# musevlt/origin

Measured on AMD Instinct MI355X. Metric: voxels/s through DCT+PCA+GLR (ORIGIN hot path), higher is better.
Workload: dtype f32+f16x2; 1 GPU; synthetic 3681x600x600 cube, Dico_FWHM_2_12 (20 profiles), PSF 25x25, 100x100 areas, dct_order 10, pfa 0.01, Noise_population 50, itermax 100; masked_border=0, glr_spectral_arithmetic=f16x2, tiles=1

## Files before the change

origin_amd/csrc/glr.hip:

```cpp
#include <algorithm>

#include "glr_plan.h"

namespace {

__global__ __launch_bounds__(256) void maxmap_final_kernel(const float *__restrict__ part_max,
                                                           const float *__restrict__ part_min,
                                                           int nzc, long S,
                                                           float *__restrict__ maxmap,
                                                           float *__restrict__ minmap) {
  const long s = (long)blockIdx.x * 256 + threadIdx.x;
  if (s >= S) return;
  float a = -INFINITY, b = INFINITY;
  for (int k = 0; k < nzc; ++k) {
    a = fmaxf(a, part_max[(long)k * S + s]);
    b = fminf(b, part_min[(long)k * S + s]);
  }
  if (maxmap) maxmap[s] = a;
  if (minmap) minmap[s] = b;
}

int launch_maxmap_final(origin_ctx *ctx, const GlrSpectralIO &io, long S, float *d_maxmap,
                        float *d_minmap) {
  hipLaunchKernelGGL(maxmap_final_kernel, dim3(cdiv(S, 256)), dim3(256), 0, ctx->stream, io.pmax,
// ... 32 lines not shown
                  GlrSpectralIO *io) {
  io->nzc = glr_part_rows(ctx, pl, form);
  io->pmax = io->want_maps ? io->part : nullptr;
  io->pmin = io->want_maps ? io->part + (size_t)io->nzc * pl->Ny * pl->Nx : nullptr;
}

int run_spectral_mfma(origin_ctx *ctx, const origin_glr_plan *pl, GlrSpectral form, bool no_fold,
                      GlrSpectralIO *io, const GlrRange &rg) {
  lay_out_maps(ctx, pl, form, io);
  if (form == GLR_SPEC_NORM_MFMA) return origin_spectral_norm_mfma_launch(ctx, pl, *io, rg);
  const bool normw = form == GLR_SPEC_NORMW;
  SpectralMfmaArgs a = glr_spectral_mfma_args(pl, io, normw || !no_fold);
  a.range = rg;
  if (!normw) return origin_spectral_mfma_launch(ctx, a);
  a.rden = a.rdi_s = a.rden_fold = a.sden = nullptr;
  a.normc = io->norm;
  if (int rc = origin_spectral_mfma_launch(ctx, a)) return rc;
  return origin_spectral_norm_mfma_launch_ends(ctx, pl, *io, rg,
                                               glr_part_rows(ctx, pl, GLR_SPEC_TABLE));
}

}

SpectralMfmaArgs glr_spectral_mfma_args(const origin_glr_plan *pl, const GlrSpectralIO *io,
                                        bool fold) {
  const bool b16 = pl->precision == 2;
  SpectralMfmaArgs a;
  a.io = io;
  a.terms = b16 ? 1 : 3;
  a.atab = b16 ? pl->d_atab_bf16 : pl->d_atab;
  a.atab_fold = !fold ? nullptr : b16 ? pl->d_atab_bf16_fold : pl->d_atab_fold;
  a.rden = pl->d_rden, a.rdi_s = pl->d_rdi_s;
  a.rden_fold = fold ? pl->d_rden_fold : nullptr, a.sden = fold ? pl->d_sden : nullptr;
  a.pinfo = pl->d_pwide;
  a.NzP = pl->NzP, a.K = pl->K, a.n_narrow = pl->n_narrow, a.ident = pl->order_ident;
  a.Nz = pl->Nz, a.Ny = pl->Ny, a.Nx = pl->Nx, a.P = pl->P;
  return a;
}

extern "C" {

int origin_glr_run_rows(origin_ctx *ctx, origin_glr_plan *pl, const float *d_cube,
                        const uint8_t *d_mask, float *d_work, float *d_correl, uint8_t *d_profile,
                        float *d_correl_min, int y0, int y1, int flags) {
  return origin_glr_run_rect(ctx, pl, d_cube, d_mask, d_work, d_correl, d_profile, d_correl_min, y0,
                             y1, 0, pl ? pl->Nx : 0, flags);
}

int origin_glr_run_rect(origin_ctx *ctx, origin_glr_plan *pl, const float *d_cube,
                        const uint8_t *d_mask, float *d_work, float *d_correl, uint8_t *d_profile,
                        float *d_correl_min, int y0, int y1, int x0, int x1, int flags) {
  ORIGIN_USE(ctx);
  ORIGIN_CHECK_ARG(pl && pl->ctx == ctx, "plan does not belong to this context");
  ORIGIN_CHECK_ARG(d_cube && d_work && d_correl && d_profile && d_correl_min, "null pointer");
  const int Ny = pl->Ny, Nx = pl->Nx;
  ORIGIN_CHECK_ARG(y0 >= 0 && y0 < y1 && y1 <= Ny && y0 % 64 == 0 && (y1 % 64 == 0 || y1 == Ny),
                   "row band must start at a multiple of 64 and end at one or at Ny");
  ORIGIN_CHECK_ARG(x0 >= 0 && x0 < x1 && x1 <= Nx && x0 % 64 == 0 && (x1 % 64 == 0 || x1 == Nx),
                   "column range must start at a multiple of 64 and end at one or at Nx");
  const bool no_fold = glr_no_fold();
  const GlrPaths paths = glr_paths(pl, no_fold);
  if (!paths.prepared) {
    origin_set_error("origin_glr_run_rows: a plan with a norm cube runs in bands after "
                     "origin_glr_plan_prepare");
    return ORIGIN_E_STATE;
  }
  if (!paths.rows_ok()) {
    origin_set_error("origin_glr_run_rows: the plan's stages do not run the matrix-core kernels");
// ... 74 lines not shown
```

origin_amd/csrc/glr_plan.h:

```cpp
#pragma once
#include <cmath>
#include <cstdlib>
#include <vector>

#include "common.h"
#include "glr_tables.h"

struct origin_glr_plan {
  origin_ctx *ctx = nullptr;
  int Nz = 0, Ny = 0, Nx = 0, nfields = 0, P = 0, K = 0;
  int mode = 0;
  int lwmax = 0;
  float *d_k = nullptr;
  float *d_k2 = nullptr;
  float *d_w = nullptr;
  float *d_taps = nullptr;
  float *d_taps2 = nullptr;
  int *d_tap_off = nullptr;
  float *d_rden = nullptr;
  int Kp = 0;
  int symmetric = 0;
  float *d_htaps = nullptr;
  int *d_htap_off = nullptr;
  float *d_rows = nullptr;
  float *d_rdi = nullptr;
  int *d_border = nullptr;
  int nborder = 0;
  int lwt = 0;
  int NzP = 0;
  uint4 *d_atab = nullptr;
  uint4 *d_atab_bf16 = nullptr;
  uint4 *d_atab2 = nullptr;
  int *d_pwide = nullptr;
  int n_narrow = 0;
  int order_ident = 0;
  float *d_rdi_s = nullptr;
  uint4 *d_atab_fold = nullptr, *d_atab_bf16_fold = nullptr;
  float *d_rden_fold = nullptr, *d_sden = nullptr;
  float fold_eps = INFINITY;
  int normw_checked = 0;
  std::vector<int> h_order;
  int precision = 0;
  float *d_normc = nullptr;
  int normc_ready = 0;
  size_t bytes = 0;
};

enum GlrSpectral {
  GLR_SPEC_TABLE,
  GLR_SPEC_NORMW,
  GLR_SPEC_NORM_MFMA,
  GLR_SPEC_PACKED,
  GLR_SPEC_FP32,
  GLR_SPEC_GENERIC
};
struct GlrPaths {
  bool spatial_mfma;
  GlrSpectral spectral;
  bool prepared;
  bool spectral_mfma() const { return spectral <= GLR_SPEC_NORM_MFMA; }
  bool rows_ok() const { return prepared && spatial_mfma && spectral_mfma(); }
};
inline bool glr_no_fold() { return getenv("ORIGIN_GLR_NO_FOLD") != nullptr; }
GlrPaths glr_paths_at(const origin_glr_plan *pl, int precision, bool no_fold);
inline GlrPaths glr_paths(const origin_glr_plan *pl, bool no_fold) {
  return glr_paths_at(pl, pl->precision, no_fold);
}

// ... 15 lines not shown

int glr_fp32_spatial(origin_ctx *ctx, const float *A, const float *B, const float *taps, int Nz,
                     int Ny, int Nx, int P, int accumulate, float *out);
struct GlrSpectralIO {
  const float *fsf, *norm;
  const uint8_t *mask;
  float *correl;
  uint8_t *profile;
  float *correl_min;
  float *part;
  bool want_maps;
  int nzc = 0;
  float *pmax = nullptr, *pmin = nullptr;
};
int glr_fp32_spectral(origin_ctx *ctx, const origin_glr_plan *pl, GlrSpectral form,
                      GlrSpectralIO *io, ProfScope *ps);
int glr_fp32_border_maps(origin_ctx *ctx, const origin_glr_plan *pl, const float *correl,
                         const float *correl_min, float *maxmap, float *minmap);

struct GlrRange {
  int y0 = 0, y1 = 0, x0 = 0, x1 = 0;
};
struct GlrSpaxels {
  long s_first, s_end, bx;
  int rx0, rx1;
};
int glr_range_resolve(const GlrRange &rg, int Ny, int Nx, int waves, GlrSpaxels *sp);
struct GlrChunks {
  int n, len;
};
GlrChunks glr_z_chunks(int num_cu, int Nz, long S, int waves);
int glr_part_rows(const origin_ctx *ctx, const origin_glr_plan *pl, GlrSpectral form);

struct SpectralMfmaArgs {
  const GlrSpectralIO *io;
  int terms;
  const uint4 *atab, *atab_fold;
  const float *rden, *rdi_s, *rden_fold, *sden;
  const int *pinfo;
  int NzP, K, n_narrow, ident;
  int Nz, Ny, Nx, P;
  GlrRange range;
  const float *normc = nullptr;
};
SpectralMfmaArgs glr_spectral_mfma_args(const origin_glr_plan *pl, const GlrSpectralIO *io,
                                        bool fold);
int origin_spectral_mfma_launch(origin_ctx *ctx, const SpectralMfmaArgs &a);
long origin_spectral_mfma_count(int num_cu, int terms, int K, int n_narrow, int Nz, int Ny,
                                int Nx);

int origin_spectral_norm_mfma_max_k();
int origin_spectral_norm_mfma_launch(origin_ctx *ctx, const origin_glr_plan *pl,
                                     const GlrSpectralIO &io, const GlrRange &rg);
int origin_spectral_norm_mfma_launch_ends(origin_ctx *ctx, const origin_glr_plan *pl,
                                          const GlrSpectralIO &io, const GlrRange &rg, int prow0);
```

origin_amd/csrc/glr_plan.hip:

```cpp
#include <algorithm>
#include <cmath>
#include <cstdlib>
#include <memory>
#include <vector>

#include "glr_plan.h"

namespace {

__global__ __launch_bounds__(256) void norm_classes_kernel(const float *__restrict__ k2, int Nz,
                                                           int P, double *__restrict__ ncls) {
  const long i = (long)blockIdx.x * 256 + threadIdx.x;
  const long n = (long)Nz * P * P;
  if (i >= n) return;
  const int z = (int)(i / (P * P));
  const int cls = (int)(i - (long)z * P * P);
  const int cy = cls / P, cx = cls - cy * P;
  const int c = P / 2;
  const int dy0 = max(0, c - cy), dy1 = min(P - 1, P - 1 + c - cy);
  const int dx0 = max(0, c - cx), dx1 = min(P - 1, P - 1 + c - cx);
  const float *kz = k2 + (long)z * P * P;
  double acc = 0.0;
  for (int dy = dy0; dy <= dy1; ++dy)
    for (int dx = dx0; dx <= dx1; ++dx) acc += (double)kz[dy * P + dx];
// ... 251 lines not shown
  };
  for (int slot = 0; slot < K; ++slot) {
    const int kk = order[slot];
    const int L = prof.len(kk), lw = prof.lw(kk);
    pinfo[slot] = kk | ((lw > 16) << 8);
    for (int c = 0; c < 8; ++c)
      for (int q = 0; q < MF_GROUPS; ++q)
        for (int j = 0; j < 8; ++j) {
          const int e = 8 * q + c + j, ti = lw + 63 - e;
          const float t = (ti >= 0 && ti < L) ? prof.taps[prof.off[kk] + ti] : 0.0f;
          const size_t base = slot * PROF + c * COPY + (size_t)q * 8 + j;
          split(t * tscale, &at[base]);
          ab[base] = to_bf16(t);
          if (!atf.empty()) {
            const float tf = (float)((double)t * (*fold_a)[kk]);
            split(tf * tscale, &atf[base]);
            abf[base] = to_bf16(tf);
          }
          if (!at2.empty()) split((t * t) * tscale, &at2[base]);
        }
  }
  origin_ctx *ctx = pl->ctx;
  if (int rc = upload(ctx, at, (_Float16 **)&pl->d_atab, &pl->bytes)) return rc;
  if (int rc = upload(ctx, ab, (unsigned short **)&pl->d_atab_bf16, &pl->bytes)) return rc;
  if (!at2.empty())
    if (int rc = upload(ctx, at2, (_Float16 **)&pl->d_atab2, &pl->bytes)) return rc;
  if (!atf.empty()) {
    if (int rc = upload(ctx, atf, (_Float16 **)&pl->d_atab_fold, &pl->bytes)) return rc;
    if (int rc = upload(ctx, abf, (unsigned short **)&pl->d_atab_bf16_fold, &pl->bytes)) return rc;
  }
  if (int rc = upload(ctx, pinfo, &pl->d_pwide, &pl->bytes)) return rc;
  pl->n_narrow = 0;
  for (int slot = 0; slot < K; ++slot) pl->n_narrow += (pinfo[slot] >> 8) == 0;
  pl->order_ident = 1;
  for (int slot = 0; slot < K; ++slot) pl->order_ident &= order[slot] == slot;
  pl->h_order = order;
  return ORIGIN_OK;
}

int alloc_norm_cube(origin_glr_plan *pl) {
  const size_t padded =
      ((size_t)pl->Nz + MF_PAD_FRONT + MF_PAD_BACK) * (size_t)pl->Ny * pl->Nx * sizeof(float);
  ORIGIN_HIP(hipMalloc((void **)&pl->d_normc, padded));
  ORIGIN_HIP(hipMemsetAsync(pl->d_normc, 0, padded, pl->ctx->stream));
  pl->bytes += padded;
  return ORIGIN_OK;
}

int build_border_tables(origin_glr_plan *pl) {
  origin_ctx *ctx = pl->ctx;
  const int Nz = pl->Nz, Ny = pl->Ny, Nx = pl->Nx, P = pl->P, K = pl->K, NzP = pl->NzP;
  const size_t PP = (size_t)P * P;
  std::vector<int> border;
  const int c = P / 2;
  for (int y = 0; y < Ny; ++y)
    for (int x = 0; x < Nx; ++x)
      if (y < c || y > Ny - 1 - c || x < c || x > Nx - 1 - c) border.push_back(y * Nx + x);
  pl->nborder = (int)border.size();
  if (int rc = upload(ctx, border, &pl->d_border, &pl->bytes)) return rc;
  DevTmp ncls;
  const size_t ncls_n = (size_t)Nz * PP, rn = PP * (size_t)K * NzP;
  ORIGIN_HIP(ncls.alloc(ncls_n * sizeof(double)));
  ORIGIN_HIP(hipMalloc((void **)&pl->d_rden, rn * sizeof(float)));
  pl->bytes += rn * sizeof(float);
  hipLaunchKernelGGL(norm_classes_kernel, dim3(cdiv((long)ncls_n, 256)), dim3(256), 0, ctx->stream,
                     pl->d_k2, Nz, P, (double *)ncls.p);
  hipLaunchKernelGGL(rden_kernel, dim3(cdiv((long)rn, 256)), dim3(256), 0, ctx->stream,
                     (const double *)ncls.p, pl->d_taps2, pl->d_tap_off, K, Nz, (int)PP, NzP,
// ... 145 lines not shown
  float *norm = pl->d_normc + (size_t)MF_PAD_FRONT * S;
  if (!pl->normc_ready) {
    ProfScope ps(ctx, K_GLR_SPATIAL);
    for (int f = 0; f < pl->nfields; ++f) {
      const float *wf = pl->d_w ? pl->d_w + (size_t)f * S : nullptr;
      const float *k2f = pl->d_k2 + (size_t)f * Nz * P * P;
      if (int rc = glr_fp32_spatial(ctx, nullptr, wf, k2f, Nz, Ny, Nx, P, f > 0, norm)) return rc;
    }
    pl->normc_ready = 1;
  }
  if (!pl->normw_checked) {
    if (pl->d_atab_fold) return measure_normw_eps(ctx, pl, norm);
    pl->normw_checked = 1;
  }
  return ORIGIN_OK;
}

extern "C" {

int origin_glr_plan_prepare(origin_ctx *ctx, origin_glr_plan *plan) {
  ORIGIN_USE(ctx);
  ORIGIN_CHECK_ARG(plan && plan->ctx == ctx, "plan does not belong to this context");
  return glr_plan_prepare(ctx, plan);
}

int origin_glr_plan_destroy(origin_glr_plan *plan) {
  if (!plan) return ORIGIN_OK;
  (void)hipSetDevice(plan->ctx->device);
  (void)hipStreamSynchronize(plan->ctx->stream);
  for (void *p : {(void *)plan->d_k, (void *)plan->d_k2, (void *)plan->d_w, (void *)plan->d_taps,
                  (void *)plan->d_taps2, (void *)plan->d_tap_off, (void *)plan->d_rden,
                  (void *)plan->d_htaps, (void *)plan->d_htap_off, (void *)plan->d_rows,
                  (void *)plan->d_border, (void *)plan->d_atab, (void *)plan->d_atab_bf16,
                  (void *)plan->d_pwide, (void *)plan->d_rdi_s, (void *)plan->d_normc,
                  (void *)plan->d_atab2, (void *)plan->d_atab_fold, (void *)plan->d_atab_bf16_fold,
                  (void *)plan->d_rden_fold, (void *)plan->d_sden})
    if (p) (void)hipFree(p);
  delete plan;
  return ORIGIN_OK;
}

int origin_glr_plan_create(origin_ctx *ctx, int Nz, int Ny, int Nx, int nfields, int P,
                           const double *h_psf, const double *h_weights, int K,
                           const double *h_taps, const int *h_tap_off,
                           origin_glr_plan **out) {
  ORIGIN_USE(ctx);
  ORIGIN_CHECK_ARG(out, "out is null");
  *out = nullptr;
  ORIGIN_CHECK_ARG(Nz > 0 && Ny > 0 && Nx > 0, "bad cube shape (%d,%d,%d)", Nz, Ny, Nx);
  ORIGIN_CHECK_ARG(nfields >= 1 && h_psf, "need at least one PSF");
  ORIGIN_CHECK_ARG(P >= 1 && (P & 1) && P <= 63, "PSF size %d unsupported (odd, <= 63)", P);
  ORIGIN_CHECK_ARG(K >= 1 && K <= 255 && h_taps && h_tap_off,
                   "need 1..255 profiles (profile index is uint8)");
  ORIGIN_CHECK_ARG(h_weights || nfields == 1, "several fields need weight maps");
  for (int k = 0; k < K; ++k)
    ORIGIN_CHECK_ARG(h_tap_off[k + 1] > h_tap_off[k], "profile %d is empty", k);

  std::unique_ptr<origin_glr_plan, PlanDeleter> owner(new origin_glr_plan());
  origin_glr_plan *pl = owner.get();
  pl->ctx = ctx;
  pl->Nz = Nz, pl->Ny = Ny, pl->Nx = Nx, pl->nfields = nfields, pl->P = P, pl->K = K;
  pl->mode = (h_weights == nullptr && Ny >= P && Nx >= P) ? 0 : 1;
  pl->NzP = (Nz + 31) / 32 * 32 + 32;
  pl->Kp = pl->NzP;

  Profiles prof;
  std::vector<double> fold_a;
// ... 18 lines not shown

int origin_glr_plan_set_precision(origin_glr_plan *plan, int precision) {
  ORIGIN_CHECK_ARG(plan && precision >= 0 && precision <= 2, "precision must be 0, 1 or 2");
  const GlrPaths at1 = glr_paths_at(plan, 1, false);
  plan->precision = at1.spatial_mfma || at1.spectral_mfma() ? precision : 0;
  return ORIGIN_OK;
}

int origin_glr_plan_get_precision(origin_glr_plan *plan, int *precision) {
  ORIGIN_CHECK_ARG(plan && precision, "null argument");
  *precision = plan->precision;
  return ORIGIN_OK;
}

int origin_glr_plan_fold_eps(origin_glr_plan *plan, float *eps, int *active) {
  ORIGIN_CHECK_ARG(plan && eps && active, "null argument");
  *eps = plan->fold_eps;
  *active = (plan->mode == 0 ? plan->d_rden_fold != nullptr
                             : plan->normw_checked && plan->d_atab_fold != nullptr &&
                                   plan->fold_eps <= MF_FOLD_EPS) &&
            !glr_no_fold();
  return ORIGIN_OK;
}

int origin_glr_plan_mfma_count(origin_glr_plan *plan, long *spatial, long *spectral) {
  ORIGIN_CHECK_ARG(plan && spatial && spectral, "null argument");
  const origin_glr_plan *pl = plan;
  *spatial = *spectral = 0;
  const GlrPaths paths = glr_paths(pl, glr_no_fold());
  const int terms = pl->precision == 2 ? 1 : 3;
  if (pl->mode == 0 && paths.spatial_mfma)
    *spatial = origin_spatial_mfma_count(terms, pl->Nz, pl->Ny, pl->Nx, pl->P);
  if (paths.spectral == GLR_SPEC_TABLE)
    *spectral = origin_spectral_mfma_count(pl->ctx->num_cu, terms, pl->K, pl->n_narrow, pl->Nz,
                                           pl->Ny, pl->Nx);
  return ORIGIN_OK;
}

int origin_glr_mfma_count_model(int num_cu, int terms, int K, int n_narrow, int Nz, int Ny, int Nx,
                                int P, long *spatial, long *spectral) {
  ORIGIN_CHECK_ARG(spatial && spectral && num_cu > 0 && (terms == 1 || terms == 3) && K > 0 &&
                       n_narrow >= 0 && n_narrow <= K && Nz > 0 && Ny > 0 && Nx > 0 && P > 0,
                   "bad arguments");
  *spatial = origin_spatial_mfma_ok(Ny, Nx, P) ? origin_spatial_mfma_count(terms, Nz, Ny, Nx, P) : 0;
  *spectral = origin_spectral_mfma_count(num_cu, terms, K, n_narrow, Nz, Ny, Nx);
  return ORIGIN_OK;
}

int origin_glr_plan_paths(origin_glr_plan *plan, int *spatial_mfma, int *spectral, int *lwt,
                          int *lwmax, int *nborder) {
  ORIGIN_CHECK_ARG(plan && spatial_mfma && spectral && lwt && lwmax && nborder, "null argument");
  const GlrPaths paths = glr_paths(plan, glr_no_fold());
  *spatial_mfma = paths.spatial_mfma ? 1 : 0;
  *spectral = (int)paths.spectral;
  *lwt = plan->lwt;
  *lwmax = plan->lwmax;
  *nborder = plan->nborder;
  return ORIGIN_OK;
}

int origin_glr_plan_bytes(origin_glr_plan *plan, size_t *bytes) {
  ORIGIN_CHECK_ARG(plan && bytes, "null argument");
  *bytes = plan->bytes;
  return ORIGIN_OK;
}

int origin_glr_work_elems(origin_glr_plan *plan, size_t *elems) {
  ORIGIN_CHECK_ARG(plan && elems, "null argument");
  *elems = GlrWork::elems(plan);
  return ORIGIN_OK;
}

int origin_glr_rows_supported(origin_glr_plan *plan, int *ok) {
  ORIGIN_CHECK_ARG(plan && ok, "null argument");
  *ok = glr_paths(plan, glr_no_fold()).rows_ok() ? 1 : 0;
  return ORIGIN_OK;
}

// ... 2 lines not shown
```

origin_amd/csrc/glr_spectral_mfma.hip:

```cpp
#include <algorithm>

#include "glr_plan.h"

namespace {

constexpr bool SM_PREFETCH = MF_WAVES <= 8;

#ifdef SM_TIMING
__device__ long long sm_wave[4 * MF_WAVES * 3];
__device__ long long sm_tim[8 * MF_WAVES * 8];
#define SM_STAMP(k)                                                                       \
  if (blockIdx.x == 3 && blockIdx.y == 1 && lane == 0 && sm_tile >= 2 && sm_tile < 10)    \
  sm_tim[((sm_tile - 2) * MF_WAVES + (threadIdx.x >> 6)) * 8 + (k)] = clock64()
#else
#define SM_STAMP(k)
#endif

typedef unsigned u32x4v __attribute__((ext_vector_type(4)));
typedef float f32x16 __attribute__((ext_vector_type(16)));
typedef float f32x4v __attribute__((ext_vector_type(4)));
typedef _Float16 f16x2v __attribute__((ext_vector_type(2)));

template <int I, int N, typename F>
__device__ __forceinline__ void sm_for(F &&f) {
// ... 47 lines not shown
        : "v"(acc[O]), "v"(acc[O + 8]), "v"(maskv), "s"(ca), "s"(cb), "s"(ninf), "s"(pinf));
    return;
  }
  if constexpr (FOLD) {
    asm volatile(
        "v_and_or_b32 %0, %5, %7, %8\n\t"
        "v_and_or_b32 %1, %6, %7, %9\n\t"
        "v_max3_f32 %2, %2, %0, %1\n\t"
        "v_max3_f32 %3, %3, %5, %6\n\t"
        "v_min3_f32 %4, %4, %5, %6"
        : "=&v"(K0), "=&v"(K1), "+v"(st.key[O]), "+v"(st.best[O]), "+v"(st.worst[O])
        : "v"(acc[O]), "v"(acc[O + 8]), "v"(maskv), "s"(ca), "s"(cb));
    return;
  }
  asm volatile(
      "v_mul_f32 %0, %7, %8\n\t"
      "v_mul_f32 %1, %9, %10\n\t"
      "v_and_or_b32 %2, %0, %11, %12\n\t"
      "v_and_or_b32 %3, %1, %11, %13\n\t"
      "v_max3_f32 %4, %4, %2, %3\n\t"
      "v_max3_f32 %5, %5, %0, %1\n\t"
      "v_min3_f32 %6, %6, %0, %1"
      : "=&v"(T0), "=&v"(T1), "=&v"(K0), "=&v"(K1), "+v"(st.key[O]), "+v"(st.best[O]),
        "+v"(st.worst[O])
      : "v"(acc[O]), "v"(fa[g][q]), "v"(acc[O + 8]), "v"(fb[g][q]), "v"(maskv), "s"(ca), "s"(cb));
}

constexpr int SM_EPI_ITEMS = 8;

constexpr int sm_epi_start(int j, int NM) {
  return j < 2 ? 0 : (j >= NM ? SM_EPI_ITEMS : (SM_EPI_ITEMS * (j - 2)) / (NM - 2));
}

template <int TERMS, int OFF, bool FOLD, int MODE = EPI_UPDATE>
__device__ __forceinline__ void sm_stage(const char *ak, const char *ak_next, u32x4v &fh,
                                         u32x4v &fl, bool wide, const u32x4v (&bh)[6],
                                         const u32x4v (&bl)[6], f32x16 &acc, const f32x16 &pacc,
                                         const f32x4v (&pfa)[2], const f32x4v (&pfb)[2],
                                         SmState &st, unsigned maskv, int pca, int pcb) {
  constexpr int LO = 8 * MF_COPY_BYTES;
  constexpr int NM = TERMS * 3;
  u32x4v ah, al;
  if constexpr (FOLD) {
    ah = fh, al = fl;
  } else {
    ah = *reinterpret_cast<const u32x4v *>(ak + 32), al = ah;
    if constexpr (TERMS == 3) al = *reinterpret_cast<const u32x4v *>(ak + 32 + LO);
  }
  sm_for<0, 3>([&](auto ic) {
    constexpr int g = decltype(ic)::value, ks = 1 + g;
    u32x4v nh = ah, nl = al;
    if constexpr (g + 1 < 3) {
      nh = *reinterpret_cast<const u32x4v *>(ak + (ks + 1) * 32);
      if constexpr (TERMS == 3) nl = *reinterpret_cast<const u32x4v *>(ak + (ks + 1) * 32 + LO);
    } else if constexpr (FOLD) {
      nh = *reinterpret_cast<const u32x4v *>(ak_next + 32), nl = nh;
      if constexpr (TERMS == 3) nl = *reinterpret_cast<const u32x4v *>(ak_next + 32 + LO);
    }
    auto gap = [&](auto jc) {
      constexpr int j = decltype(jc)::value;
      sm_for<sm_epi_start(j, NM), sm_epi_start(j + 1, NM)>([&](auto kc) {
        sm_epi_item<decltype(kc)::value, FOLD, MODE>(pacc, pfa, pfb, st, maskv, pca, pcb);
      });
    };
    sm_mma<TERMS, g == 0>(acc, ah, bh[OFF + ks]);
    gap(std::integral_constant<int, TERMS * g>{});
    if constexpr (TERMS == 3) {
      sm_mma<TERMS, false>(acc, ah, bl[OFF + ks]);
      gap(std::integral_constant<int, TERMS * g + 1>{});
      sm_mma<TERMS, false>(acc, al, bh[OFF + ks]);
      gap(std::integral_constant<int, TERMS * g + 2>{});
    }
    ah = nh, al = nl;
  });
  if constexpr (FOLD) fh = ah, fl = al;
  if (wide) {
    const u32x4v a0h = *reinterpret_cast<const u32x4v *>(ak);
    const u32x4v a4h = *reinterpret_cast<const u32x4v *>(ak + 4 * 32);
    if constexpr (TERMS == 3) {
      const u32x4v a0l = *reinterpret_cast<const u32x4v *>(ak + LO);
      const u32x4v a4l = *reinterpret_cast<const u32x4v *>(ak + 4 * 32 + LO);
      sm_mma<TERMS, false>(acc, a0h, bh[OFF + 0]);
      sm_mma<TERMS, false>(acc, a0h, bl[OFF + 0]);
      sm_mma<TERMS, false>(acc, a0l, bh[OFF + 0]);
      sm_mma<TERMS, false>(acc, a4h, bh[OFF + 4]);
      sm_mma<TERMS, false>(acc, a4h, bl[OFF + 4]);
      sm_mma<TERMS, false>(acc, a4l, bh[OFF + 4]);
    } else {
      sm_mma<TERMS, false>(acc, a0h, bh[OFF + 0]);
      sm_mma<TERMS, false>(acc, a4h, bh[OFF + 4]);
    }
  }
}

template <bool FOLD>
__device__ __forceinline__ void sm_drain(const f32x16 &pacc, const f32x4v (&pfa)[2],
                                         const f32x4v (&pfb)[2], SmState &st, unsigned maskv,
                                         int pca, int pcb) {
  unsigned mv = maskv;
  asm volatile("s_nop 15\n\ts_nop 3" : "+v"(mv));
  sm_for<0, SM_EPI_ITEMS>([&](auto kc) {
    sm_epi_item<decltype(kc)::value, FOLD>(pacc, pfa, pfb, st, mv, pca, pcb);
  });
}

template <int TERMS, bool BW, bool PODD, bool FOLD, bool IDENT = false, bool NORMW = false>
__device__ __forceinline__ void sm_tiles(
    const float *__restrict__ sdl, const float *__restrict__ fsf, const float *__restrict__ rdb, const float *__restrict__ rdi_s,
    int NzP, const int *__restrict__ pinfo, int K, int NP, int Nz, long S, long s_base, int rr,
    bool sv, bool all_valid, int h, int lane, const char *a_lane, char *rd_wave, int zc0, int zc1,
    const uint8_t *__restrict__ mask, float *__restrict__ correl, uint8_t *__restrict__ profile,
    float *__restrict__ correl_min, float &vmax, float &vmin, int nN, char *stage = nullptr) {
  const char *rd_lane = rd_wave + 16 * h;
  const bool second = (lane & 16) != 0;
  const unsigned off_in = 4u * ((unsigned)(8 * h * S) + rr);
  const unsigned off_out = (unsigned)(4 * h * S) + rr;
  const unsigned off_out4 = 4u * off_out;
  const unsigned off_rd = 4u * (unsigned)((lane >> 5) * NzP + (lane & 31));
  auto ldf = [](const float *base, unsigned boff) {
    return *reinterpret_cast<const float *>(reinterpret_cast<const char *>(base) + boff);
  };
  auto stf = [](float *base, unsigned boff, float v) {
    *reinterpret_cast<float *>(reinterpret_cast<char *>(base) + boff) = v;
  };
// ... 221 lines not shown
            mk[i] = (mask + (long)zu * S + s_base)[(unsigned)rr + (h ? hs : 0u)];
          }
        }
      }
      f32x4v sg[2] = {(f32x4v){0.f, 0.f, 0.f, 0.f}, (f32x4v){0.f, 0.f, 0.f, 0.f}};
      if constexpr (FOLD && NORMW) {
        const float *qp = sdl + (long)zh * S + s_base;
        unsigned on4 = off_out4;
        SM_PIN(on4);
#pragma unroll
        for (int i = 0; i < 8; ++i) {
          sg[i >> 2][i & 3] = ldf(qp, on4);
          qp += (i & 3) == 3 ? 5 * S : S;
        }
      } else if constexpr (FOLD) {
#pragma unroll
        for (int g = 0; g < 2; ++g) sg[g] = *reinterpret_cast<const f32x4v *>(sdl + zh + 8 * g);
      }
      SmState st;
      if constexpr (!FOLD) {
#pragma unroll
        for (int i = 0; i < 8; ++i)
          st.best[i] = -INFINITY, st.worst[i] = INFINITY, st.key[i] = -INFINITY;
      }

      f32x16 accX, accY;
      f32x4v fa[2], fb[2];
      int ca = 0, cb = 0;
#pragma unroll
      for (int g = 0; g < 2; ++g) fa[g] = fb[g] = (f32x4v){NAN, NAN, NAN, NAN};
      asm volatile("s_nop 1" : "=v"(accY));
      const char *akp = a_lane + (second ? MF_PROF_BYTES : 0);
      u32x4v fh, fl;
      if constexpr (FOLD) {
        fh = *reinterpret_cast<const u32x4v *>(akp + 32), fl = fh;
        if constexpr (TERMS == 3) fl = *reinterpret_cast<const u32x4v *>(akp + 32 + 8 * MF_COPY_BYTES);
      }
      auto run = [&](int p, f32x16 &wacc, const f32x16 &racc, auto mode_c) {
        constexpr int MODE = decltype(mode_c)::value;
        const int sa = 2 * p, sb = min(2 * p + 1, K - 1);
        int ia, ib;
        if constexpr (IDENT) {
          ia = sa, ib = sb | (sb >= nN ? 0x100 : 0);
        } else {
          ia = pinfo[sa], ib = pinfo[sb];
        }
        const char *ak = akp;
        akp += 2 * MF_PROF_BYTES;
        sm_stage<TERMS, HALF, FOLD, MODE>(ak, akp, fh, fl, ((ia | ib) >> 8) != 0, bh, bl, wacc,
                                          racc, fa, fb, st, maskv, ca, cb);
        const int ka = ia & 0xff, kb = ib & 0xff;
        if constexpr (FOLD) {
        } else if constexpr (BW) {
#pragma unroll
          for (int g = 0; g < 2; ++g) {
            fa[g] = *reinterpret_cast<const f32x4v *>(rdb + (long)ka * NzP + zh + 8 * g);
            fb[g] = *reinterpret_cast<const f32x4v *>(rdb + (long)kb * NzP + zh + 8 * g);
          }
        } else {
#pragma unroll
          for (int g = 0; g < 2; ++g) {
            fa[g] = *reinterpret_cast<const f32x4v *>(rd_lane + sa * MF_RD_BYTES + 64 * HALF + 32 * g);
            fb[g] = *reinterpret_cast<const f32x4v *>(rd_lane + sb * MF_RD_BYTES + 64 * HALF + 32 * g);
          }
        }
        ca = 31 - ka, cb = 31 - kb;
      };
      using UpdC = std::integral_constant<int, EPI_UPDATE>;
      int p = 0;
      if constexpr (FOLD) {
        run(0, accX, accY, std::integral_constant<int, EPI_NONE>{});
        run(1, accY, accX, std::integral_constant<int, EPI_FIRST>{});
        p = 2;
      }
      for (; p + 1 < NP; p += 2) {
        run(p, accX, accY, UpdC{});
        run(p + 1, accY, accX, UpdC{});
      }
      SM_STAMP(2 + 3 * HALF);
      if constexpr (PODD) {
        run(p, accX, accY, UpdC{});
        sm_drain<FOLD>(accX, fa, fb, st, maskv, ca, cb);
      } else {
        sm_drain<FOLD>(accY, fa, fb, st, maskv, ca, cb);
      }
      SM_STAMP(3 + 3 * HALF);

      auto store = [&](auto straight_c) {
        constexpr bool STRAIGHT = decltype(straight_c)::value;
        float *cp = correl + (long)zh * S + s_base, *np = correl_min + (long)zh * S + s_base;
        uint8_t *pp = profile + (long)zh * S + s_base;
        unsigned oo = off_out, oo4 = off_out4;
        if constexpr (STRAIGHT) {
          SM_PIN(oo);
          SM_PIN(oo4);
        }
#pragma unroll
        for (int i = 0; i < 8; ++i) {
          const int zu = zh + (i & 3) + 8 * (i >> 2);
          if (STRAIGHT || zu + 4 * h < zc1) {
            float f = inv;
            if constexpr (FOLD && NORMW) {
              const float nv = sg[i >> 2][i & 3];
              f = nv > 0.0f ? __builtin_amdgcn_rsqf(nv) * inv : 0.0f;
            } else if constexpr (FOLD) {
              f = sg[i >> 2][i & 3] * inv;
            }
            float b = st.best[i] * f;
            float w = st.worst[i] * f;
            int kk = 31 - (int)(__float_as_uint(st.key[i]) & 31u);
            if (st.best[i] == st.worst[i]) kk = 0;
            if (mk[i]) b = 0.0f, kk = 0;
            if (STRAIGHT || sv) {
              stf(cp, oo4, b);
              stf(np, oo4, w);
              pp[oo] = (uint8_t)kk;
            }
            vmax = fmaxf(vmax, b);
// ... 85 lines not shown
      if (a < b)
        sm_tiles<TERMS, true, PODD, false>(nullptr, fsf, rdb, rdi_s, NzP, pinfo, K, NP, Nz, S,
                                           s_base, rr, sv, all_valid, h, lane, a_lane, rd_wave, a, b,
                                           mask, correl, profile, correl_min, vmax, vmin, nN);
    }
  } else if (__any(cls != ccls)) {
    sm_tiles<TERMS, true, PODD, false>(nullptr, fsf, rdb, rdi_s, NzP, pinfo, K, NP, Nz, S, s_base,
                                       rr, sv, all_valid, h, lane, a_lane, rd_wave, zc0, zc1, mask,
                                       correl, profile, correl_min, vmax, vmin, nN);
  } else {
    sm_tiles<TERMS, false, PODD, false>(nullptr, fsf, rdb, rdi_s, NzP, pinfo, K, NP, Nz, S, s_base,
                                        rr, sv, all_valid, h, lane, a_lane, rd_wave, zc0, zc1, mask,
                                        correl, profile, correl_min, vmax, vmin, nN);
  }
  if (part_max) {
    const float a = fmaxf(vmax, __shfl_xor(vmax, 32));
    const float b = fminf(vmin, __shfl_xor(vmin, 32));
    if (h == 0 && sv) {
      part_max[(long)blockIdx.y * S + sc] = a;
      part_min[(long)blockIdx.y * S + sc] = b;
    }
  }
  }
#ifdef SM_TIMING
  if (sm_rec) {
    sm_wave[((blockIdx.x - 3) * MF_WAVES + wv) * 3 + 1] = clock64();
    sm_wave[((blockIdx.x - 3) * MF_WAVES + wv) * 3 + 2] = wall_clock64() - sm_wall0;
  }
#endif
}

}

long origin_spectral_mfma_count(int num_cu, int terms, int K, int n_narrow, int Nz, int Ny,
                                int Nx) {
  const long S = (long)Ny * Nx;
  const GlrChunks zc = glr_z_chunks(num_cu, Nz, S, MF_WAVES);
  long tiles = 0;
  for (int c = 0; c < zc.n; ++c) tiles += cdiv(std::min(zc.len, Nz - c * zc.len), 32);
  long ksteps = 0;
  for (int p = 0; p < (K + 1) / 2; ++p) {
    const int sb = std::min(2 * p + 1, K - 1);
    ksteps += sb >= n_narrow ? 5 : 3;
  }
  const long waves = cdiv(S, 32);
  return waves * tiles * 2 * ksteps * terms;
}

int origin_spectral_mfma_launch(origin_ctx *ctx, const SpectralMfmaArgs &a) {
  const GlrSpectralIO *io = a.io;
  const int K = a.K, Nz = a.Nz, Nx = a.Nx;
  const GlrChunks zc = glr_z_chunks(ctx->num_cu, Nz, (long)a.Ny * Nx, MF_WAVES);
  GlrSpaxels sp;
  if (int rc = glr_range_resolve(a.range, a.Ny, Nx, MF_WAVES, &sp)) return rc;
  const int Kp = K + (K & 1);
  const size_t lds = std::max((size_t)Kp * MF_PROF_BYTES + (size_t)K * MF_WAVES * MF_RD_BYTES,
                              (size_t)(Kp + 1) * MF_PROF_BYTES);
  const int NP = (K + 1) / 2;
  auto pick = [&](int fold) -> const void * {
    const int variant = (NP & 1) | (fold << 1) | ((fold && a.ident) << 2) | ((fold && a.normc) << 3);
#define SM_PICK(T, V) \
  if (a.terms == T && variant == V) return (const void *)spectral_mfma2_kernel<T, V>
    SM_PICK(3, 0); SM_PICK(3, 1); SM_PICK(3, 2); SM_PICK(3, 3); SM_PICK(3, 6); SM_PICK(3, 7);
    SM_PICK(1, 0); SM_PICK(1, 1); SM_PICK(1, 2); SM_PICK(1, 3); SM_PICK(1, 6); SM_PICK(1, 7);
    SM_PICK(3, 10); SM_PICK(3, 11); SM_PICK(3, 14); SM_PICK(3, 15);
    SM_PICK(1, 10); SM_PICK(1, 11); SM_PICK(1, 14); SM_PICK(1, 15);
#undef SM_PICK
    return nullptr;
  };
  int zf0 = 0, zf1 = 0;
  if (a.atab_fold && ((a.rden_fold && a.sden) || a.normc)) mf_fold_range(Nz, &zf0, &zf1);
  const size_t lds_fold = (size_t)Kp * MF_PROF_BYTES + (size_t)MF_WAVES * MF_STAGE_BYTES;
  if (!mf_fold_fits(K) || NP < 2) zf0 = zf1 = 0;
  const int fold = zf1 > zf0;
  const void *fn = pick(fold);
  if (!fn) {
    origin_set_error("spectral MFMA kernel: no variant for %d terms", a.terms);
    return ORIGIN_E_STATE;
  }
  if (a.normc && !fold) {
    origin_set_error("spectral MFMA kernel: the norm-cube form needs the FOLD range");
    return ORIGIN_E_STATE;
  }
  ORIGIN_HIP(hipFuncSetAttribute(fn, hipFuncAttributeMaxDynamicSharedMemorySize,
                                 MF_MAX_K * (MF_PROF_BYTES + MF_WAVES * MF_RD_BYTES)));
  const float *fsf = io->fsf, *k_rden = fold ? a.rden_fold : a.rden, *rdi_s = a.rdi_s;
  const float *k_sden = fold && a.normc ? a.normc : a.sden;
  const uint4 *k_atab = fold ? a.atab_fold : a.atab;
  const int *pinfo = a.pinfo;
  const uint8_t *mask = io->mask;
  float *correl = io->correl, *correl_min = io->correl_min;
  uint8_t *profile = io->profile;
  float *pmax = io->pmax, *pmin = io->pmin;
  int NzP = a.NzP, k_K = K, k_NP = NP, k_Nz = Nz, Ny = a.Ny, k_Nx = Nx, P = a.P, k_zcm = zc.len;
  int nN = a.n_narrow;
  void *args[] = {&fsf, &k_rden, &rdi_s, &NzP, &k_atab, &pinfo, &k_K, &k_NP, &k_Nz, &Ny, &k_Nx, &P,
                  &k_zcm, &mask, &correl, &profile, &correl_min, &pmax, &pmin, &k_sden, &zf0, &zf1,
                  &nN, &sp.s_first, &sp.s_end, &sp.rx0, &sp.rx1};
  ORIGIN_HIP(hipLaunchKernel(fn, dim3((unsigned)sp.bx, (unsigned)zc.n), dim3(64 * MF_WAVES), args,
                             fold ? std::max(lds, lds_fold) : lds, ctx->stream));
  ORIGIN_LAUNCH_CHECK();
  return ORIGIN_OK;
}

#ifdef SM_TIMING
extern "C" int origin_debug_sm_timing(long long *out) {
  return (int)hipMemcpyFromSymbol(out, HIP_SYMBOL(sm_tim), sizeof(long long) * 8 * MF_WAVES * 8);
}
extern "C" int origin_debug_sm_waves(long long *out) {
  return (int)hipMemcpyFromSymbol(out, HIP_SYMBOL(sm_wave), sizeof(long long) * 4 * MF_WAVES * 3);
}
#endif
```

Baseline: 26.95 billion voxels/s.

## Split spectral MFMA profile pairs into four width classes to skip k-steps

Replaces the two-way narrow/wide profile split with four classes by line width (≤8, ≤16, ≤24, wider). Each pair now issues 2 to 5 MFMA k-steps instead of 3 or 5. DPP lane swaps on the B blocks and a per-half offset let partial k-steps reuse the same fragments, so narrow profiles skip the zero-band MFMAs. The cost is extra DPP swaps, s_nop hazard padding, more branching and a new class table in the plan.

New measurement: 26.69 billion voxels/s. Within noise of the previous version (-1.0%).

```diff
diff --git a/origin_amd/csrc/glr.hip b/origin_amd/csrc/glr.hip
--- a/origin_amd/csrc/glr.hip
+++ b/origin_amd/csrc/glr.hip
@@ -88,8 +88,8 @@
   a.atab_fold = !fold ? nullptr : b16 ? pl->d_atab_bf16_fold : pl->d_atab_fold;
   a.rden = pl->d_rden, a.rdi_s = pl->d_rdi_s;
   a.rden_fold = fold ? pl->d_rden_fold : nullptr, a.sden = fold ? pl->d_sden : nullptr;
-  a.pinfo = pl->d_pwide;
-  a.NzP = pl->NzP, a.K = pl->K, a.n_narrow = pl->n_narrow, a.ident = pl->order_ident;
+  a.pinfo = pl->d_pclass;
+  a.NzP = pl->NzP, a.K = pl->K, a.class_bounds = pl->class_bounds, a.ident = pl->order_ident;
   a.Nz = pl->Nz, a.Ny = pl->Ny, a.Nx = pl->Nx, a.P = pl->P;
   return a;
 }
diff --git a/origin_amd/csrc/glr_plan.h b/origin_amd/csrc/glr_plan.h
--- a/origin_amd/csrc/glr_plan.h
+++ b/origin_amd/csrc/glr_plan.h
@@ -33,7 +33,10 @@
   uint4 *d_atab2 = nullptr;
   int *d_pwide = nullptr;
   int n_narrow = 0;
+  int *d_pclass = nullptr;
+  std::vector<int> h_class;
   int order_ident = 0;
+  int class_bounds = 0;
   float *d_rdi_s = nullptr;
   uint4 *d_atab_fold = nullptr, *d_atab_bf16_fold = nullptr;
   float *d_rden_fold = nullptr, *d_sden = nullptr;
@@ -115,13 +118,16 @@
 GlrChunks glr_z_chunks(int num_cu, int Nz, long S, int waves);
 int glr_part_rows(const origin_ctx *ctx, const origin_glr_plan *pl, GlrSpectral form);
 
+inline int mf_class(int lw) { return lw <= 8 ? 0 : lw <= 16 ? 1 : lw <= 24 ? 2 : 3; }
+constexpr int mf_class_ksteps(int c) { return 2 + c; }
+constexpr int mf_class_mask(int c) { return (1 << c) - 1; }
 struct SpectralMfmaArgs {
   const GlrSpectralIO *io;
   int terms;
   const uint4 *atab, *atab_fold;
   const float *rden, *rdi_s, *rden_fold, *sden;
   const int *pinfo;
-  int NzP, K, n_narrow, ident;
+  int NzP, K, class_bounds, ident;
   int Nz, Ny, Nx, P;
   GlrRange range;
   const float *normc = nullptr;
@@ -129,7 +135,7 @@
 SpectralMfmaArgs glr_spectral_mfma_args(const origin_glr_plan *pl, const GlrSpectralIO *io,
                                         bool fold);
 int origin_spectral_mfma_launch(origin_ctx *ctx, const SpectralMfmaArgs &a);
-long origin_spectral_mfma_count(int num_cu, int terms, int K, int n_narrow, int Nz, int Ny,
+long origin_spectral_mfma_count(int num_cu, int terms, int K, const int *kclass, int Nz, int Ny,
                                 int Nx);
 
 int origin_spectral_norm_mfma_max_k();
diff --git a/origin_amd/csrc/glr_plan.hip b/origin_amd/csrc/glr_plan.hip
--- a/origin_amd/csrc/glr_plan.hip
+++ b/origin_amd/csrc/glr_plan.hip
@@ -307,8 +307,19 @@
   if (int rc = upload(ctx, pinfo, &pl->d_pwide, &pl->bytes)) return rc;
   pl->n_narrow = 0;
   for (int slot = 0; slot < K; ++slot) pl->n_narrow += (pinfo[slot] >> 8) == 0;
+  std::vector<int> pclass(K);
+  pl->h_class.assign(K, 0);
+  int nle[3] = {0, 0, 0};
   pl->order_ident = 1;
-  for (int slot = 0; slot < K; ++slot) pl->order_ident &= order[slot] == slot;
+  for (int slot = 0; slot < K; ++slot) {
+    const int c = mf_class(prof.lw(order[slot]));
+    pl->h_class[slot] = c;
+    pclass[slot] = order[slot] | (mf_class_mask(c) << 8);
+    for (int b = c; b < 3; ++b) ++nle[b];
+    pl->order_ident &= order[slot] == slot && (slot == 0 || c >= pl->h_class[slot - 1]);
+  }
+  pl->class_bounds = nle[0] | (nle[1] << 8) | (nle[2] << 16);
+  if (int rc = upload(ctx, pclass, &pl->d_pclass, &pl->bytes)) return rc;
   pl->h_order = order;
   return ORIGIN_OK;
 }
@@ -520,7 +531,8 @@
                   (void *)plan->d_taps2, (void *)plan->d_tap_off, (void *)plan->d_rden,
                   (void *)plan->d_htaps, (void *)plan->d_htap_off, (void *)plan->d_rows,
                   (void *)plan->d_border, (void *)plan->d_atab, (void *)plan->d_atab_bf16,
-                  (void *)plan->d_pwide, (void *)plan->d_rdi_s, (void *)plan->d_normc,
+                  (void *)plan->d_pwide, (void *)plan->d_pclass, (void *)plan->d_rdi_s,
+                  (void *)plan->d_normc,
                   (void *)plan->d_atab2, (void *)plan->d_atab_fold, (void *)plan->d_atab_bf16_fold,
                   (void *)plan->d_rden_fold, (void *)plan->d_sden})
     if (p) (void)hipFree(p);
@@ -605,18 +617,23 @@
   if (pl->mode == 0 && paths.spatial_mfma)
     *spatial = origin_spatial_mfma_count(terms, pl->Nz, pl->Ny, pl->Nx, pl->P);
   if (paths.spectral == GLR_SPEC_TABLE)
-    *spectral = origin_spectral_mfma_count(pl->ctx->num_cu, terms, pl->K, pl->n_narrow, pl->Nz,
-                                           pl->Ny, pl->Nx);
+    *spectral = origin_spectral_mfma_count(pl->ctx->num_cu, terms, pl->K, pl->h_class.data(),
+                                           pl->Nz, pl->Ny, pl->Nx);
   return ORIGIN_OK;
 }
 
 int origin_glr_mfma_count_model(int num_cu, int terms, int K, int n_narrow, int Nz, int Ny, int Nx,
                                 int P, long *spatial, long *spectral) {
+  const int n_le16 = n_narrow & 0xff, n_le8 = (n_narrow >> 8) & 0xff, n_17_24 = (n_narrow >> 16) & 0xff;
   ORIGIN_CHECK_ARG(spatial && spectral && num_cu > 0 && (terms == 1 || terms == 3) && K > 0 &&
-                       n_narrow >= 0 && n_narrow <= K && Nz > 0 && Ny > 0 && Nx > 0 && P > 0,
+                       n_narrow >= 0 && (n_narrow >> 24) == 0 && n_le8 <= n_le16 &&
+                       n_le16 + n_17_24 <= K && Nz > 0 && Ny > 0 && Nx > 0 && P > 0,
                    "bad arguments");
+  std::vector<int> kclass(K);
+  for (int slot = 0; slot < K; ++slot)
+    kclass[slot] = slot < n_le8 ? 0 : slot < n_le16 ? 1 : slot < n_le16 + n_17_24 ? 2 : 3;
   *spatial = origin_spatial_mfma_ok(Ny, Nx, P) ? origin_spatial_mfma_count(terms, Nz, Ny, Nx, P) : 0;
-  *spectral = origin_spectral_mfma_count(num_cu, terms, K, n_narrow, Nz, Ny, Nx);
+  *spectral = origin_spectral_mfma_count(num_cu, terms, K, kclass.data(), Nz, Ny, Nx);
   return ORIGIN_OK;
 }
 
diff --git a/origin_amd/csrc/glr_spectral_mfma.hip b/origin_amd/csrc/glr_spectral_mfma.hip
--- a/origin_amd/csrc/glr_spectral_mfma.hip
+++ b/origin_amd/csrc/glr_spectral_mfma.hip
@@ -103,64 +103,82 @@
   return j < 2 ? 0 : (j >= NM ? SM_EPI_ITEMS : (SM_EPI_ITEMS * (j - 2)) / (NM - 2));
 }
 
+template <int TERMS>
+__device__ __forceinline__ void sm_swap_low_lanes(u32x4v &xh, u32x4v &xl, u32x4v &yh, u32x4v &yl) {
+  auto sw = [](u32x4v &x, u32x4v &y) {
+#pragma unroll
+    for (int j = 0; j < 4; ++j) {
+      const int t = (int)x[j];
+      x[j] = (unsigned)__builtin_amdgcn_update_dpp(t, (int)y[j], 0xE4, 0x3, 0xf, false);
+      y[j] = (unsigned)__builtin_amdgcn_update_dpp((int)y[j], t, 0xE4, 0x3, 0xf, false);
+    }
+  };
+  sw(xh, yh);
+  if constexpr (TERMS == 3) sw(xl, yl);
+  if constexpr (TERMS == 3) asm volatile("s_nop 1" : "+v"(xh), "+v"(yh), "+v"(xl), "+v"(yl));
+  else asm volatile("s_nop 1" : "+v"(xh), "+v"(yh));
+}
+
 template <int TERMS, int OFF, bool FOLD, int MODE = EPI_UPDATE>
 __device__ __forceinline__ void sm_stage(const char *ak, const char *ak_next, u32x4v &fh,
-                                         u32x4v &fl, bool wide, const u32x4v (&bh)[6],
+                                         u32x4v &fl, int t, unsigned m64, const u32x4v (&bh)[6],
                                          const u32x4v (&bl)[6], f32x16 &acc, const f32x16 &pacc,
                                          const f32x4v (&pfa)[2], const f32x4v (&pfb)[2],
                                          SmState &st, unsigned maskv, int pca, int pcb) {
   constexpr int LO = 8 * MF_COPY_BYTES;
-  constexpr int NM = TERMS * 3;
-  u32x4v ah, al;
-  if constexpr (FOLD) {
-    ah = fh, al = fl;
-  } else {
-    ah = *reinterpret_cast<const u32x4v *>(ak + 32), al = ah;
-    if constexpr (TERMS == 3) al = *reinterpret_cast<const u32x4v *>(ak + 32 + LO);
-  }
-  sm_for<0, 3>([&](auto ic) {
-    constexpr int g = decltype(ic)::value, ks = 1 + g;
+  constexpr int NM = TERMS * 2;
+  auto frag = [](const char *q, u32x4v &xh, u32x4v &xl) {
+    xh = *reinterpret_cast<const u32x4v *>(q), xl = xh;
+    if constexpr (TERMS == 3) xl = *reinterpret_cast<const u32x4v *>(q + LO);
+  };
+  auto bare = [&](const u32x4v &qh, const u32x4v &ql, const u32x4v &xh, const u32x4v &xl) {
+    sm_mma<TERMS, false>(acc, qh, xh);
+    if constexpr (TERMS == 3) {
+      sm_mma<TERMS, false>(acc, qh, xl);
+      sm_mma<TERMS, false>(acc, ql, xh);
+    }
+  };
+  const unsigned mo = t == 0 ? m64 : 0u;
+  u32x4v ah, al, ch, cl;
+  if constexpr (FOLD) ah = fh, al = fl;
+  else frag(ak + 2 * 32, ah, al);
+  sm_for<0, 2>([&](auto ic) {
+    constexpr int g = decltype(ic)::value;
     u32x4v nh = ah, nl = al;
-    if constexpr (g + 1 < 3) {
-      nh = *reinterpret_cast<const u32x4v *>(ak + (ks + 1) * 32);
-      if constexpr (TERMS == 3) nl = *reinterpret_cast<const u32x4v *>(ak + (ks + 1) * 32 + LO);
-    } else if constexpr (FOLD) {
-      nh = *reinterpret_cast<const u32x4v *>(ak_next + 32), nl = nh;
-      if constexpr (TERMS == 3) nl = *reinterpret_cast<const u32x4v *>(ak_next + 32 + LO);
+    if constexpr (g == 0) {
+      frag(ak + mo + 32, nh, nl);
+    } else {
+      frag(ak + 3 * 32, ch, cl);
+      if constexpr (FOLD) frag(ak_next + 2 * 32, nh, nl);
     }
     auto gap = [&](auto jc) {
       constexpr int j = decltype(jc)::value;
+      if constexpr (NM == 2 && j == 1 && MODE != EPI_NONE) asm volatile("s_nop 15");
       sm_for<sm_epi_start(j, NM), sm_epi_start(j + 1, NM)>([&](auto kc) {
         sm_epi_item<decltype(kc)::value, FOLD, MODE>(pacc, pfa, pfb, st, maskv, pca, pcb);
       });
     };
-    sm_mma<TERMS, g == 0>(acc, ah, bh[OFF + ks]);
+    sm_mma<TERMS, g == 0>(acc, ah, bh[OFF + 2 - g]);
     gap(std::integral_constant<int, TERMS * g>{});
     if constexpr (TERMS == 3) {
-      sm_mma<TERMS, false>(acc, ah, bl[OFF + ks]);
+      sm_mma<TERMS, false>(acc, ah, bl[OFF + 2 - g]);
       gap(std::integral_constant<int, TERMS * g + 1>{});
-      sm_mma<TERMS, false>(acc, al, bh[OFF + ks]);
+      sm_mma<TERMS, false>(acc, al, bh[OFF + 2 - g]);
       gap(std::integral_constant<int, TERMS * g + 2>{});
     }
     ah = nh, al = nl;
   });
   if constexpr (FOLD) fh = ah, fl = al;
-  if (wide) {
-    const u32x4v a0h = *reinterpret_cast<const u32x4v *>(ak);
-    const u32x4v a4h = *reinterpret_cast<const u32x4v *>(ak + 4 * 32);
-    if constexpr (TERMS == 3) {
-      const u32x4v a0l = *reinterpret_cast<const u32x4v *>(ak + LO);
-      const u32x4v a4l = *reinterpret_cast<const u32x4v *>(ak + 4 * 32 + LO);
-      sm_mma<TERMS, false>(acc, a0h, bh[OFF + 0]);
-      sm_mma<TERMS, false>(acc, a0h, bl[OFF + 0]);
-      sm_mma<TERMS, false>(acc, a0l, bh[OFF + 0]);
-      sm_mma<TERMS, false>(acc, a4h, bh[OFF + 4]);
-      sm_mma<TERMS, false>(acc, a4h, bl[OFF + 4]);
-      sm_mma<TERMS, false>(acc, a4l, bh[OFF + 4]);
-    } else {
-      sm_mma<TERMS, false>(acc, a0h, bh[OFF + 0]);
-      sm_mma<TERMS, false>(acc, a4h, bh[OFF + 4]);
-    }
+  if (t & 1) bare(ch, cl, bh[OFF + 3], bl[OFF + 3]);
+  if (t & 2) {
+    u32x4v qh, ql;
+    frag(ak + ((t & 4) ? 0u : 2 * m64), qh, ql);
+    bare(qh, ql, bh[OFF + 0], bl[OFF + 0]);
+  }
+  if (t & 4) {
+    u32x4v rh, rl;
+    frag(ak + 4 * 32, rh, rl);
+    bare(rh, rl, bh[OFF + 4], bl[OFF + 4]);
   }
 }
 
@@ -448,23 +466,36 @@
       asm volatile("s_nop 1" : "=v"(accY));
       const char *akp = a_lane + (second ? MF_PROF_BYTES : 0);
       u32x4v fh, fl;
-      if constexpr (FOLD) {
-        fh = *reinterpret_cast<const u32x4v *>(akp + 32), fl = fh;
-        if constexpr (TERMS == 3) fl = *reinterpret_cast<const u32x4v *>(akp + 32 + 8 * MF_COPY_BYTES);
-      }
+      auto pair_info = [&](int p, int &ia, int &ib) {
+        const int sa = 2 * p, sb = min(2 * p + 1, K - 1);
+        if constexpr (IDENT) {
+          const int c = (sb >= (nN & 0xff)) + (sb >= ((nN >> 8) & 0xff)) + (sb >= (nN >> 16));
+          ia = sa, ib = sb | (((1 << c) - 1) << 8);
+        } else {
+          ia = pinfo[sa], ib = pinfo[sb];
+        }
+      };
+      int swapped = 0;
+      auto swap_blocks = [&](int m) {
+        if (m & 1) sm_swap_low_lanes<TERMS>(bh[HALF + 1], bl[HALF + 1], bh[HALF + 3], bl[HALF + 3]);
+        if (m & 2) sm_swap_low_lanes<TERMS>(bh[HALF + 0], bl[HALF + 0], bh[HALF + 4], bl[HALF + 4]);
+      };
+      unsigned m64 = h ? 0u : 64u;
+      SM_PIN(m64);
       auto run = [&](int p, f32x16 &wacc, const f32x16 &racc, auto mode_c) {
         constexpr int MODE = decltype(mode_c)::value;
         const int sa = 2 * p, sb = min(2 * p + 1, K - 1);
         int ia, ib;
-        if constexpr (IDENT) {
-          ia = sa, ib = sb | (sb >= nN ? 0x100 : 0);
-        } else {
-          ia = pinfo[sa], ib = pinfo[sb];
-        }
+        pair_info(p, ia, ib);
+        const int t = (ia | ib) >> 8;
+        const int want = t == 0 ? 1 : (t == 3 ? 2 : 0);
+        swap_blocks(swapped ^ want);
+        swapped = want;
+        if constexpr (TERMS == 1) asm volatile("s_nop 1" : "+v"(bh[HALF + 1]));
         const char *ak = akp;
         akp += 2 * MF_PROF_BYTES;
-        sm_stage<TERMS, HALF, FOLD, MODE>(ak, akp, fh, fl, ((ia | ib) >> 8) != 0, bh, bl, wacc,
-                                          racc, fa, fb, st, maskv, ca, cb);
+        sm_stage<TERMS, HALF, FOLD, MODE>(ak, akp, fh, fl, t, m64, bh, bl, wacc, racc, fa, fb, st,
+                                          maskv, ca, cb);
         const int ka = ia & 0xff, kb = ib & 0xff;
         if constexpr (FOLD) {
         } else if constexpr (BW) {
@@ -482,6 +513,10 @@
         }
         ca = 31 - ka, cb = 31 - kb;
       };
+      if constexpr (FOLD) {
+        fh = *reinterpret_cast<const u32x4v *>(akp + 64), fl = fh;
+        if constexpr (TERMS == 3) fl = *reinterpret_cast<const u32x4v *>(akp + 64 + 8 * MF_COPY_BYTES);
+      }
       using UpdC = std::integral_constant<int, EPI_UPDATE>;
       int p = 0;
       if constexpr (FOLD) {
@@ -494,12 +529,10 @@
         run(p + 1, accY, accX, UpdC{});
       }
       SM_STAMP(2 + 3 * HALF);
-      if constexpr (PODD) {
-        run(p, accX, accY, UpdC{});
-        sm_drain<FOLD>(accX, fa, fb, st, maskv, ca, cb);
-      } else {
-        sm_drain<FOLD>(accY, fa, fb, st, maskv, ca, cb);
-      }
+      if constexpr (PODD) run(p, accX, accY, UpdC{});
+      swap_blocks(swapped);
+      if constexpr (PODD) sm_drain<FOLD>(accX, fa, fb, st, maskv, ca, cb);
+      else sm_drain<FOLD>(accY, fa, fb, st, maskv, ca, cb);
       SM_STAMP(3 + 3 * HALF);
 
       auto store = [&](auto straight_c) {
@@ -651,7 +684,7 @@
 
 }
 
-long origin_spectral_mfma_count(int num_cu, int terms, int K, int n_narrow, int Nz, int Ny,
+long origin_spectral_mfma_count(int num_cu, int terms, int K, const int *kclass, int Nz, int Ny,
                                 int Nx) {
   const long S = (long)Ny * Nx;
   const GlrChunks zc = glr_z_chunks(num_cu, Nz, S, MF_WAVES);
@@ -660,7 +693,7 @@
   long ksteps = 0;
   for (int p = 0; p < (K + 1) / 2; ++p) {
     const int sb = std::min(2 * p + 1, K - 1);
-    ksteps += sb >= n_narrow ? 5 : 3;
+    ksteps += mf_class_ksteps(std::max(kclass[2 * p], kclass[sb]));
   }
   const long waves = cdiv(S, 32);
   return waves * tiles * 2 * ksteps * terms;
@@ -712,7 +745,7 @@
   uint8_t *profile = io->profile;
   float *pmax = io->pmax, *pmin = io->pmin;
   int NzP = a.NzP, k_K = K, k_NP = NP, k_Nz = Nz, Ny = a.Ny, k_Nx = Nx, P = a.P, k_zcm = zc.len;
-  int nN = a.n_narrow;
+  int nN = a.class_bounds;
   void *args[] = {&fsf, &k_rden, &rdi_s, &NzP, &k_atab, &pinfo, &k_K, &k_NP, &k_Nz, &Ny, &k_Nx, &P,
                   &k_zcm, &mask, &correl, &profile, &correl_min, &pmax, &pmin, &k_sden, &zf0, &zf1,
                   &nN, &sp.s_first, &sp.s_end, &sp.rx0, &sp.rx1};
```
